# quinnchr-personal/Continuum-Mechanics-MFEM

Measured on AMD Instinct MI355X. Metric: DoF-iter/s (CG, 3D p=2 hex convection-diffusion) + achieved HBM GB/s, higher is better.
Workload: dtype f64; 1 GPU; 64x64x64 hex, H1 p=2, PA D+C+M (kinds=7), Jacobi-CG 100 it/step; dofs=2146689, elements=262144, parallelism=single, series=weak: an n^3 slab per rank

## Files before the change

### continuum-mechanics-mfem_amd/csrc/brick_core.hpp

```cpp
#pragma once
#include <hip/hip_runtime.h>

#include <cstdint>
#include <type_traits>

#include "pa_core.hpp"

#ifndef CDFEM_PS8_SKIP
#define CDFEM_PS8_SKIP 1
#endif

namespace cdfem {

struct BrickGeom {
    int nbx, nby, nbz;
    int Lx, Ly, Lz;
    int xcd;
    int bz0, bzs;
    const uint8_t *bess;
    int stag = 0, stag_round = 0;
};

__device__ __forceinline__ void brick_stagger(const BrickGeom &g)
{
// ... 45 lines not shown
template <int S, int STEP = 64>
struct LatWalk {
    int x, y, z;
    uint32_t gid;
    __device__ __forceinline__ LatWalk(unsigned t, uint32_t g0, uint32_t Lx, uint32_t Lxy)
        : x((int)(t % S)), y((int)((t / S) % S)), z((int)(t / (S * S)))
    {
        gid = g0 + (uint32_t)x + Lx * (uint32_t)y + Lxy * (uint32_t)z;
    }
    __device__ __forceinline__ void next(uint32_t dgid, uint32_t cxd, uint32_t cyd)
    {
        constexpr int dx = STEP % S, dy = (STEP / S) % S, dz = STEP / (S * S);
        x += dx;
        const int cx = x >= S ? 1 : 0;
        x -= S & -cx;
        y += dy + cx;
        const int cy = y >= S ? 1 : 0;
        y -= S & -cy;
        z += dz + cy;
        gid += dgid + (cxd & (uint32_t)-cx) + (cyd & (uint32_t)-cy);
    }
};

template <int B, int E, typename F>
__device__ __forceinline__ void static_for(F &&f)
{
    if constexpr (B < E) {
        f(std::integral_constant<int, B>{});
        static_for<B + 1, E>(f);
    }
}

__device__ __forceinline__ int opaque(int v)
{
    asm volatile("" : "+v"(v));
    return v;
}

template <int S, int SZ = S>
__device__ __forceinline__ double patch_sum8(__amdgpu_buffer_rsrc_t bp, const BrickGeom &g, int gx, int gy, int gz)
{
    constexpr int s1 = S - 1, sz1 = SZ - 1;
    const int qx = min(gx / s1, g.nbx - 1), qy = min(gy / s1, g.nby - 1), qz = min(gz / sz1, g.nbz - 1);
    const int px = gx - qx * s1, py = gy - qy * s1, pz = gz - qz * sz1;
    const bool fx = px == 0 && qx > 0, fy = py == 0 && qy > 0, fz = pz == 0 && qz > 0;
    const uint32_t R = (uint32_t)g.nbx * S, A = (uint32_t)g.nby * S * R;
// ... 42 lines not shown
```

### continuum-mechanics-mfem_amd/csrc/brick_kernels.hip

```cpp
#include <hip/hip_runtime.h>

#include <type_traits>
#include <vector>
#include <algorithm>
#include <cmath>

#include "cdfem_internal.hpp"
#include "brick_core.hpp"
#include "pa_core.hpp"
#include "reduce.hpp"

#ifndef CDFEM_BRICK_LDS
#define CDFEM_BRICK_LDS 1
#endif

namespace cdfem {

__device__ __forceinline__ int bsel(bool c, int a, int b)
{
    const int m = -(int)c;
    return (a & m) | (b & ~m);
}
template <int S>
__device__ __forceinline__ int face_index(int a, int b, int c)
// ... 580 lines not shown
    }
    den = wave_sum(den);
    if (grp <= 1) {
        if (t == 0) part[b] = den;
        return;
    }
    const int gi = b / grp, g0 = gi * grp, gn = min(grp, nbrick - g0);
    uint32_t prev = 0;
    if (t == 0) {
        __hip_atomic_store(&part[b], den, __ATOMIC_RELAXED, __HIP_MEMORY_SCOPE_AGENT);
        asm volatile("s_waitcnt vmcnt(0)" ::: "memory");
        prev = __hip_atomic_fetch_add(&gcnt[gi], 1u, __ATOMIC_RELAXED, __HIP_MEMORY_SCOPE_AGENT);
    }
    prev = (uint32_t)__shfl((int)prev, 0, 64);
    if (prev != (uint32_t)(gn - 1)) return;
    double v = t < gn ? __hip_atomic_load(&part[g0 + t], __ATOMIC_RELAXED, __HIP_MEMORY_SCOPE_AGENT) : 0.0;
    v = wave_sum(v);
    if (t == 0) {
        gsum[gi] = v;
        __hip_atomic_store(&gcnt[gi], 0u, __ATOMIC_RELAXED, __HIP_MEMORY_SCOPE_AGENT);
    }
}

template <int S, bool XF, bool PB = false, bool DS = false, bool EP = false, int SZ = S>
__global__ void __launch_bounds__(kRedThreads)
k_cg_update_faces(double *__restrict__ x, double *__restrict__ r, const double *__restrict__ d,
                  const double *__restrict__ dinv, const double *__restrict__ pb,
                  const uint8_t *__restrict__ ess, const BrickGeom g,
                  const FastDiv fdx, const FastDiv fdxy, int zlo_shared,
                  const double *__restrict__ remote_lo, const double *__restrict__ remote_hi,
                  double *__restrict__ part, KrylovState *__restrict__ st, int den_step,
                  const double *__restrict__ apart, int napart)
{
    constexpr int s1 = S - 1, sz1 = SZ - 1;
    constexpr uint32_t PV = (uint32_t)S * S * SZ;
    __shared__ double sh[kRedThreads / 64 + 1];
    if (st->done) return;
    double alpha = 0.0;
    if constexpr (DS) {
        const double den = sum_partials_all<16>(apart, napart, sh);
        if (blockIdx.x == 0 && threadIdx.x == 0) cg_den_step(st, den);
        if (den == 0.0) return;
        alpha = st->betanom / den;
    } else if (den_step) {
        const double den = st->red[0];
        if (blockIdx.x == 0 && threadIdx.x == 0) cg_den_step(st, den);
        if (den == 0.0) return;
        alpha = st->betanom / den;
    } else {
        alpha = st->alpha;
    }
    const int n = g.Lx * g.Ly * g.Lz;
    const int plane = g.Lx * g.Ly;
    double acc = 0.0;
    if constexpr (EP) {
        static_assert(PB, "EP reads the patch buffer with the predicated loads");
        const auto bp = brsrc(pb, 8u * (uint32_t)g.nbx * g.nby * g.nbz * PV);
        for (int gid = blockIdx.x * blockDim.x + threadIdx.x; gid < n; gid += gridDim.x * blockDim.x) {
            const int gz = (int)fdiv((uint32_t)gid, fdxy);
            const int rem = gid - gz * plane;
            const int gy = (int)fdiv((uint32_t)rem, fdx);
            const int gx = rem - gy * g.Lx;
            const double rold = r[gid], mi = dinv[gid];
            const double xi = XF ? 0.0 : x[gid], di = XF ? 0.0 : d[gid];
            double qi = patch_sum8<S, SZ>(bp, g, gx, gy, gz);
            if (remote_lo && gz == 0) qi += remote_lo[rem];
            if (remote_hi && gz == g.Lz - 1) qi += remote_hi[rem];
            if constexpr (!XF) __builtin_nontemporal_store(xi + alpha * di, &x[gid]);
            const double ri = rold - alpha * qi;
            __builtin_nontemporal_store(ri, &r[gid]);
            if (!(zlo_shared && gz == 0)) acc += ri * (mi * ri);
        }
    } else {
        for (int gid = blockIdx.x * blockDim.x + threadIdx.x; gid < n; gid += gridDim.x * blockDim.x) {
            const int gz = (int)fdiv((uint32_t)gid, fdxy);
            const int rem = gid - gz * plane;
            const int gy = (int)fdiv((uint32_t)rem, fdx);
            const int gx = rem - gy * g.Lx;
            const bool is_ess = ess[gid] != 0;
            const double di = (!XF || is_ess) ? d[gid] : 0.0, xi = XF ? 0.0 : x[gid];
            const double rold = r[gid], mi = dinv[gid];
            double qi;
            if constexpr (PB) {
                qi = patch_sum8<S, SZ>(brsrc(pb, 8u * (uint32_t)g.nbx * g.nby * g.nbz * PV), g, gx, gy, gz);
            } else if (gx % s1 == 0 || gy % s1 == 0 || gz % sz1 == 0) {
                int bxs[2], pxs[2], nxc = 0, bys[2], pys[2], nyc = 0, bzs[2], pzs[2], nzc = 0;
                const int qx = gx / s1, qy = gy / s1, qz = gz / sz1;
                if (gx - qx * s1 == 0) {
                    if (qx - 1 >= 0) { bxs[nxc] = qx - 1; pxs[nxc] = s1; ++nxc; }
                    if (qx < g.nbx) { bxs[nxc] = qx; pxs[nxc] = 0; ++nxc; }
                } else { bxs[0] = qx; pxs[0] = gx - qx * s1; nxc = 1; }
                if (gy - qy * s1 == 0) {
                    if (qy - 1 >= 0) { bys[nyc] = qy - 1; pys[nyc] = s1; ++nyc; }
                    if (qy < g.nby) { bys[nyc] = qy; pys[nyc] = 0; ++nyc; }
                } else { bys[0] = qy; pys[0] = gy - qy * s1; nyc = 1; }
                if (gz - qz * sz1 == 0) {
                    if (qz - 1 >= 0) { bzs[nzc] = qz - 1; pzs[nzc] = sz1; ++nzc; }
                    if (qz < g.nbz) { bzs[nzc] = qz; pzs[nzc] = 0; ++nzc; }
                } else { bzs[0] = qz; pzs[0] = gz - qz * sz1; nzc = 1; }
                qi = 0.0;
                for (int kz = 0; kz < nzc; ++kz)
                    for (int ky = 0; ky < nyc; ++ky)
                        for (int kx = 0; kx < nxc; ++kx) {
                            qi += pb[patch_idx<S, SZ>(g, bxs[kx], bys[ky], bzs[kz], pxs[kx], pys[ky], pzs[kz])];
// ... 431 lines not shown
    BrickRun edge{0, c->nbz - 1, 2, s}, inner{1, 1, c->nbz - 2, c->stream};
    if (bfkk >= 0) {
        edge.kk = inner.kk = bfkk;
        edge.nupart = inner.nupart = cg_den_fold_grid(c);
    }
    const hipError_t e = brick_cg2_run(c, r, dinv, d_old, d_new, q, edge, x);
    if (e != hipSuccess) return e;
    return brick_cg2_run(c, r, dinv, d_old, d_new, q, inner, x);
}

hipError_t launch_cg_update_faces(cdfem_ctx *c, double *x, double *r, const double *q, const double *d,
                                  const double *dinv, const double *remote_lo, const double *remote_hi,
                                  bool den_step, bool xfold)
{
    const BrickGeom g = geom_of(c);
    const FastDiv fdx = make_fastdiv((uint32_t)c->Lx), fdxy = make_fastdiv((uint32_t)(c->Lx * c->Ly));
    const int64_t need = (c->nl + kRedThreads - 1) / kRedThreads;
    const unsigned grid = (unsigned)(need < 16384 ? need : 16384);
    const bool ds = !den_step && cg_den_fold_on(c);
    const unsigned ugrid = ds ? (unsigned)cg_den_fold_grid(c) : grid;
    double *const upart = ds ? c->d_part + c->nblk : c->d_part;
    const double *const apart = c->den_grp > 1 ? c->d_gsum : c->d_part;
    const int napart = c->den_grp > 1 ? den_parts(c) : c->nblk;
#define CDFEM_UPD4(S_, XF_, PB_, DS_, EP_)                                                                 \
    hipLaunchKernelGGL((k_cg_update_faces<S_, XF_, PB_, DS_, EP_, SZ_>), dim3(ugrid), dim3(kRedThreads), 0, c->stream, x, \
                       r, d, dinv, c->d_face, c->d_ess, g, fdx, fdxy, c->zlo_shared, remote_lo, remote_hi, upart, \
                       c->d_state, (int)den_step, apart, napart)
    const bool ep = pa_af(c) == 2 && c->p <= 2;
#define CDFEM_UPD3(S_, XF_, PB_, DS_)                                                                      \
    if (ep && PB_) { CDFEM_UPD4(S_, XF_, PB_, DS_, PB_); } else { CDFEM_UPD4(S_, XF_, PB_, DS_, false); }
#define CDFEM_UPD2(S_, XF_, PB_)                                                                           \
    if (ds) { CDFEM_UPD3(S_, XF_, PB_, true); } else { CDFEM_UPD3(S_, XF_, PB_, false); }
    const bool pb = c->brick_upd_pb != 0 && brick_fits(c);
#define CDFEM_UPD(S_)                                                                                       \
    if (xfold) {                                                                                            \
        if (pb) { CDFEM_UPD2(S_, true, true); } else { CDFEM_UPD2(S_, true, false); }                       \
    } else {                                                                                                \
        if (pb) { CDFEM_UPD2(S_, false, true); } else { CDFEM_UPD2(S_, false, false); }                     \
    }
    if (c->p == 1) {
        constexpr int SZ_ = kBrick * 1 + 1;
        CDFEM_UPD(kBrick * 1 + 1);
    } else if (c->p == 2 || (c->p == 4 && c->hb_ez == 2)) {
        constexpr int SZ_ = kBrick * 2 + 1;
        CDFEM_UPD(kBrick * 2 + 1);
    } else if (c->p == 4 && c->hb_ez == 4) {
        constexpr int SZ_ = 4 * 4 + 1;
        CDFEM_UPD(kHoBrickEdge * 4 + 1);
    } else if (c->p == 3 && c->hb_ez == 2) {
        constexpr int SZ_ = kHoBrickEdge * 3 + 1;
        CDFEM_UPD(kHoBrickEdge * 3 + 1);
    } else if (c->p == 3 && c->hb_ez == 4) {
        constexpr int SZ_ = 4 * 3 + 1;
        CDFEM_UPD(kHoBrickEdge * 3 + 1);
    } else {
        return hipErrorInvalidValue;
// ... 81 lines not shown
```

### continuum-mechanics-mfem_amd/csrc/brick_um.hip

```cpp
#include <hip/hip_runtime.h>

#include <algorithm>
#include <cmath>
#include <vector>

#include "cdfem_internal.hpp"
#include "brick_core.hpp"
#include "pa_core.hpp"
#include "reduce.hpp"

#ifndef CDFEM_BUM_ADD
#define CDFEM_BUM_ADD 0
#endif

namespace cdfem {

constexpr int kUmSlots = 32, kUmN = 27;
constexpr int kUmRow[kUmSlots] = {0,  1,  4,  3,  2,  7,  22, 5,  6,  19, 10, 21, 8,  25, 16, 23,
                                  18, 9,  12, 13, 20, 11, 14, -1, 24, 15, -1, -1, 26, 17, -1, -1};
constexpr int um_class(int l) { return (l % 3 & 1) | ((l / 3 % 3 & 1) << 1) | ((l / 9 & 1) << 2); }
constexpr bool um_row_order_ok()
{
    int seen[kUmN] = {};
    for (int g = 0; g < kUmSlots / 4; ++g) {
// ... 5 lines not shown
            if (l >= kUmN || seen[l]++) return false;
            if (cls & (1 << um_class(l))) return false;
            cls |= 1 << um_class(l);
        }
    }
    for (int l = 0; l < kUmN; ++l)
        if (!seen[l]) return false;
    return true;
}
static_assert(um_row_order_ok(), "kUmRow: every dof once, one class once per group of 4 slots");

template <int G>
__device__ __forceinline__ int um_slot_off(int kg)
{
    constexpr int S = 9;
    auto off = [](int l) constexpr { return l < 0 ? -1 : (l / 9) * S * S + (l / 3 % 3) * S + l % 3; };
    constexpr int o0 = off(kUmRow[4 * G]), o1 = off(kUmRow[4 * G + 1]), o2 = off(kUmRow[4 * G + 2]),
                  o3 = off(kUmRow[4 * G + 3]);
    return kg == 0 ? o0 : kg == 1 ? o1 : kg == 2 ? o2 : o3;
}
template <int G>
constexpr bool um_group_padded() { return kUmRow[4 * G + 1] < 0 || kUmRow[4 * G + 2] < 0 || kUmRow[4 * G + 3] < 0; }

template <bool XF, bool BF, bool FULL>
__global__ void __launch_bounds__(64, 2)
k_brick_cg(const double *__restrict__ r, const double *__restrict__ dinv, const double *__restrict__ d_old,
           double *__restrict__ d_new, double *__restrict__ face, const double *__restrict__ amat,
           const uint8_t *__restrict__ ess, const BrickGeom g, int zlo_shared, double *__restrict__ part,
           KrylovState *__restrict__ st, double *__restrict__ x, const double *__restrict__ upart, int nupart,
           int kk, double *__restrict__ gsum, uint32_t *__restrict__ gcnt, int grp, int nbrick)
{
    constexpr int P = 2, S = kBrick * P + 1, S2 = S * S, S3 = S * S * S, NDE = kUmN;
    static_assert(S == 9, "um_slot_off is written for the 9^3 patch");
    __shared__ double s_in[S3];
    __shared__ double s_out[S3];
    if (st->done) return;
    brick_stagger(g);
    double beta = st->beta;
    constexpr int NPL = 16;
    double pv[NPL];
    if constexpr (BF) {
        if (kk > 0) {
            const auto bu = brsrc(upart, 8u * (uint32_t)nupart);
#pragma unroll
            for (int i = 0; i < NPL; ++i) pv[i] = bload(bu, 8u * ((uint32_t)threadIdx.x + 64u * i));
        }
    }
    const double alpha_prev = XF ? st->alpha : 0.0;
    const int t = threadIdx.x;
    const int bl = brick_id(g), nxy = g.nbx * g.nby;
    const int bz = g.bz0 + (bl / nxy) * g.bzs;
    const int b = bl % nxy + nxy * bz;
    const int bx = b % g.nbx, by = (b / g.nbx) % g.nby;
    const int gx0 = (S - 1) * bx, gy0 = (S - 1) * by, gz0 = (S - 1) * bz;
    const bool lastx = bx == g.nbx - 1, lasty = by == g.nby - 1, lastz = bz == g.nbz - 1;
    double den = 0.0;
    constexpr int NI = (S3 + 63) / 64;
    const int Lx = g.Lx, Lxy = g.Lx * g.Ly;
    const uint32_t nl = (uint32_t)Lxy * (uint32_t)g.Lz;
    const auto br = brsrc(r, 8u * nl), bm = brsrc(dinv, 8u * nl), bo = brsrc(d_old, 8u * nl);
    const auto be = brsrc(ess, nl), bd = brsrc(d_new, 8u * nl), bxf = brsrc(x, XF ? 8u * nl : 0u);
    double rv[NI], mv[NI], ov[NI], xv[NI];
    uint32_t woffv[NI];
    uint32_t dbits = 0, ebits = 0;
    uint8_t ev[NI];
    double dev[NI];
    const uint32_t uLx = (uint32_t)Lx, uLxy = (uint32_t)Lxy;
    constexpr uint32_t wdx = 64 % S, wdy = (64 / S) % S, wdz = 64 / (S * S);
    const uint32_t dgid = wdx + wdy * uLx + wdz * uLxy, cxd = uLx - S, cyd = uLxy - S * uLx;
    LatWalk<S> pw0(t, (uint32_t)gx0 + uLx * (uint32_t)gy0 + uLxy * (uint32_t)gz0, uLx, uLxy);
    auto gather = [&](auto kc) {
        constexpr int k = decltype(kc)::value;
        const unsigned i = t + 64 * k;
        const int px = pw0.x, py = pw0.y, pz = pw0.z;
        const uint32_t gid = pw0.gid;
        pw0.next(dgid, cxd, cyd);
        const int gz = gz0 + pz;
        const bool in = i < S3 && (FULL || (gx0 + px < g.Lx && gy0 + py < g.Ly && gz < g.Lz));
        const uint32_t off = in ? 8u * gid : kOOB;
        rv[k] = bload(br, off);
        mv[k] = bload(bm, off);
        ov[k] = bload(bo, off);
        ev[k] = __builtin_amdgcn_raw_buffer_load_b8(be, in ? gid : kOOB, 0, 0);
        const bool writer = in && (px < S - 1 || lastx) && (py < S - 1 || lasty) && (pz < S - 1 || lastz);
        woffv[k] = writer ? off : kOOB;
        dbits |= (uint32_t)(writer && !(zlo_shared && gz == 0)) << k;
        if constexpr (XF) xv[k] = bload(bxf, woffv[k]);
    };
    auto form = [&](auto kc) {
        constexpr int k = decltype(kc)::value;
        const unsigned i = t + 64 * k;
        if (k == NI - 1 && i >= S3) return;
        const double dn = mv[k] * rv[k] + beta * ov[k];
        const bool e = ev[k] != 0;
        bstore(bd, woffv[k], dn);
        if constexpr (XF) bstore(bxf, woffv[k], xv[k] + alpha_prev * ov[k]);
        den += (e && ((dbits >> k) & 1u)) ? dn * dn : 0.0;
        s_in[i] = e ? 0.0 : dn;
        s_out[i] = 0.0;
        ebits |= (uint32_t)e << k;
        dev[k] = ((dbits >> k) & 1u) ? dn : 0.0;
    };
    static_for<0, NI>(gather);
    if constexpr (BF) {
        if (kk > 0) {
            double v = 0.0;
#pragma unroll
            for (int q = 0; q < NPL; ++q) v += pv[q];
            const double B = wave_sum(v);
            const bool stop = cg_stop_kind(st, B, kk) != kCgGoOn;
            if (b == 0 && t == 0) {
#ifdef CDFEM_DEBUG
                assert(st->iter == kk);
#endif
                cg_update_logic_at(st, B, kk);
            }
            if (stop) return;
            beta = B / st->nom;
        }
    }
    static_for<0, NI>(form);
    __syncthreads();

    {
        const int n16 = t & 15, kg = t >> 4;
        double av[2][7];
#pragma unroll
        for (int mt = 0; mt < 2; ++mt)
#pragma unroll
            for (int ks = 0; ks < 7; ++ks) av[mt][ks] = amat[(mt * 7 + ks) * 64 + t];
        const int ob0 = P * (n16 >> 2) * S + P * (n16 & 3);
        const bool vxy = FULL || (gx0 + P * (n16 & 3) + P < g.Lx && gy0 + P * (n16 >> 2) + P < g.Ly);
        auto node_off = [&](int j) { return (j / 9) * S2 + ((j / 3) % 3) * S + j % 3; };
        v4d_t acc[2][4];
#pragma unroll
        for (int mt = 0; mt < 2; ++mt)
#pragma unroll
            for (int nt = 0; nt < 4; ++nt) acc[mt][nt] = v4d_t{0.0, 0.0, 0.0, 0.0};
#pragma unroll
        for (int ks = 0; ks < 7; ++ks) {
            const int j = 4 * ks + kg;
            const int jo = node_off(j < NDE ? j : 0);
#pragma unroll
// ... 64 lines not shown
        __hip_atomic_store(&part[b], den, __ATOMIC_RELAXED, __HIP_MEMORY_SCOPE_AGENT);
        asm volatile("s_waitcnt vmcnt(0)" ::: "memory");
        prev = __hip_atomic_fetch_add(&gcnt[gi], 1u, __ATOMIC_RELAXED, __HIP_MEMORY_SCOPE_AGENT);
    }
    prev = (uint32_t)__shfl((int)prev, 0, 64);
    if (prev != (uint32_t)(gn - 1)) return;
    double v = t < gn ? __hip_atomic_load(&part[g0 + t], __ATOMIC_RELAXED, __HIP_MEMORY_SCOPE_AGENT) : 0.0;
    v = wave_sum(v);
    if (t == 0) {
        gsum[gi] = v;
        __hip_atomic_store(&gcnt[gi], 0u, __ATOMIC_RELAXED, __HIP_MEMORY_SCOPE_AGENT);
    }
}

hipError_t launch_brick_um(cdfem_ctx *c, const BrickGeom &g, unsigned nbrick_launch, hipStream_t s, bool whole,
                           const double *r, const double *dinv, const double *d_old, double *d_new, double *x, int kk,
                           int nupart)
{
    if (c->d_uelem == nullptr || c->p != 2) return hipErrorInvalidValue;
    const dim3 grid(nbrick_launch), block(64);
    const double *upart = c->d_part + c->nblk;
    double *const dpart = c->den_out ? c->den_out : c->d_part;
    const bool full = c->sx % kBrick == 0 && c->sy % kBrick == 0 && c->sz % kBrick == 0;
#define CDFEM_BUM(XF_, BF_, FU_)                                                                              \
    do {                                                                                                      \
        if (whole)                                                                                            \
            CDFEM_LAUNCH(c, (k_brick_cg<XF_, BF_, FU_>), grid, block, 0, r, dinv, d_old, d_new, c->d_face,      \
                         c->d_uelem, c->d_ess, g, c->zlo_shared, dpart, c->d_state, x, upart, nupart, kk,       \
                         c->d_gsum, c->d_gcnt, c->den_grp, c->nblk);                                            \
        else                                                                                                  \
            hipLaunchKernelGGL((k_brick_cg<XF_, BF_, FU_>), grid, block, 0, s, r, dinv, d_old, d_new, c->d_face, \
                               c->d_uelem, c->d_ess, g, c->zlo_shared, dpart, c->d_state, x, upart, nupart, kk, \
                               c->d_gsum, c->d_gcnt, c->den_grp, c->nblk);                                      \
    } while (0)
#define CDFEM_BUM2(XF_, BF_)                                                                                  \
    do {                                                                                                      \
        if (full) CDFEM_BUM(XF_, BF_, true);                                                                  \
        else CDFEM_BUM(XF_, BF_, false);                                                                      \
    } while (0)
    if (kk >= 0) {
        if (x) CDFEM_BUM2(true, true);
        else CDFEM_BUM2(false, true);
    } else {
        if (x) CDFEM_BUM2(true, false);
        else CDFEM_BUM2(false, false);
    }
#undef CDFEM_BUM2
#undef CDFEM_BUM
    return hipGetLastError();
}

__global__ void __launch_bounds__(256)
k_uniform_check(const double *__restrict__ gaff, const int32_t *__restrict__ perm, int nslots, int nc, int ne,
                double tol, int *__restrict__ bad)
{
    const int s = blockIdx.x * blockDim.x + threadIdx.x;
    if (s >= nslots) return;
    const int e = perm[s];
    if (e < 0 || e >= ne) return;
    const size_t b = (size_t)(s / kLanes), lane = (size_t)(s % kLanes);
    bool diff = false;
    for (int k = 0; k < nc; ++k) diff |= fabs(gaff[(b * nc + k) * kLanes + lane] - gaff[(size_t)k * kLanes]) > tol;
    if (diff) *bad = 1;
}

template <int D1, int Q1, unsigned K>
__global__ void __launch_bounds__(64)
k_uniform_elem(const double *__restrict__ gaff, const Tab<D1, Q1> T, double *__restrict__ A)
{
    constexpr int N = D1 * D1 * D1;
// ... 49 lines not shown
        if (e == hipSuccess) e = hipStreamSynchronize(c->stream);
    }
    const hipError_t ef = hipFree(scratch);
    if (e != hipSuccess) return e;
    if (ef != hipSuccess) return ef;
    if (hbad) return hipSuccess;
    for (int mt = 0; mt < 2; ++mt)
        for (int ks = 0; ks < 7; ++ks)
            for (int l = 0; l < 64; ++l) {
                const int i = kUmRow[16 * mt + (l & 15)], j = 4 * ks + (l >> 4);
                op[(mt * 7 + ks) * 64 + l] = (i >= 0 && j < N) ? h[i * N + j] : 0.0;
            }
    void *d = nullptr;
    if ((e = hipMalloc(&d, sizeof(double) * op.size())) != hipSuccess) return e;
    e = hipMemcpy(d, op.data(), sizeof(double) * op.size(), hipMemcpyHostToDevice);
    if (e != hipSuccess) {
        (void)hipFree(d);
        return e;
    }
    c->d_uelem = static_cast<double *>(d);
    return hipSuccess;
}

}
```

### continuum-mechanics-mfem_amd/csrc/capi.hip

```cpp
#include <hip/hip_runtime.h>

#include <algorithm>
#include <chrono>
#include <cmath>
#include <cstdio>
#include <cstdlib>
#include <cstring>
#include <limits>
#include <new>
#include <stdexcept>
#include <string>
#include <vector>

#include "cdfem_internal.hpp"
#include "brick_core.hpp"

using namespace cdfem;

namespace {

struct HipError : std::runtime_error {
    explicit HipError(const std::string &m) : std::runtime_error(m) {}
};
struct ArgError : std::runtime_error {
// ... 83 lines not shown
                for (int k = 0; k < dim; ++k)
                    if (v >> k & 1) p += X[(1 << k) * dim + i] - X[i];
                if (std::fabs(p - X[v * dim + i]) > tol) return false;
            }
        }
    }
    return true;
}

void free_mesh(cdfem_ctx *c)
{
    dfree(c->d_verts); dfree(c->d_map); dfree(c->d_e2l_off); dfree(c->d_e2l_pos);
    dfree(c->d_ess); dfree(c->d_ess_list); dfree(c->d_qd); dfree(c->d_qaff); dfree(c->d_geom); dfree(c->d_hgeom); dfree(c->d_Ye); dfree(c->d_dinv);
    for (auto &w : c->d_w) dfree(w);
    dfree(c->d_part); dfree(c->d_tpart); dfree(c->d_gm); dfree(c->d_gm_part); dfree(c->d_ktab);
    c->ktab_key = -1;
    dfree(c->d_perm); dfree(c->d_face); dfree(c->d_ones); dfree(c->d_dalt);
    for (auto &b : c->d_if) dfree(b);
    dfree(c->d_stab); dfree(c->d_stab_lf); dfree(c->d_rowptr); dfree(c->d_cols); dfree(c->d_diagpos); dfree(c->d_coff);
    dfree(c->d_cpos); dfree(c->d_vals); dfree(c->d_vals_c); dfree(c->d_Ee);
    dfree(c->d_sptr); dfree(c->d_srows); dfree(c->d_scols); dfree(c->d_smap); dfree(c->d_sdel); dfree(c->d_svals);
    dfree(c->d_swide);
    dfree(c->d_uelem);
    dfree(c->d_hoelem);
    c->d_sdel = nullptr;
    c->d_swide = nullptr;
    c->sell_nnz_wide = 0;
    dfree(c->d_hptr); dfree(c->d_hidx); dfree(c->d_sloc);
    c->d_hptr = c->d_hidx = nullptr;
    c->d_sloc = nullptr;
    c->lds_rows = 0;
    c->lds_max = 0;
    c->sell_lpr = 1;
    dfree(c->d_rperm); dfree(c->d_pv[0]); dfree(c->d_pv[1]); dfree(c->d_dinv_p);
    c->d_rperm = nullptr; c->d_pv[0] = c->d_pv[1] = nullptr; c->d_dinv_p = nullptr;
    dfree(c->d_svals_c);
    c->d_svals_c = nullptr;
    dfree(c->d_lfq);
    c->lfq_cap = 0;
    ilu_free(c);
    partition_free(c);
    c->nslices = c->nstored = 0;
    c->sell_windowed = false;
    c->geom = 0;
    c->fa_ready = false;
    c->nnz = 0;
// ... 209 lines not shown
void dev_out(cdfem_ctx *c, double *dst, int where, const double *dsrc, size_t n)
{
    if (where == CDFEM_DEVICE) {
        if (dst != dsrc)
            HIPCHK(hipMemcpyAsync(dst, dsrc, n * sizeof(double), hipMemcpyDeviceToDevice, c->stream));
        return;
    }
    HIPCHK(hipMemcpyAsync(dst, dsrc, n * sizeof(double), hipMemcpyDeviceToHost, c->stream));
    HIPCHK(hipStreamSynchronize(c->stream));
}

void ensure_dinv(cdfem_ctx *c)
{
    if (c->dinv_ready) return;
    double *diag = c->d_w[7];
    if (c->fa_ready) {
        HIPCHK(launch_csr_diag(c, diag));
    } else {
        HIPCHK(launch_diag_elem(c, c->d_Ye));
        HIPCHK(launch_e2l(c, c->d_Ye, nullptr, diag, false, 0));
    }
    interface_sum(c, diag);
    HIPCHK(launch_dinv(c, diag, c->d_dinv));
    c->dinv_ready = true;
}

const double *solver_dinv(cdfem_ctx *c)
{
    ensure_dinv(c);
    if (!c->perm_space) return c->d_dinv;
    if (!c->d_dinv_p) c->d_dinv_p = dalloc<double>(c->nl);
    HIPCHK(launch_perm(c, true, c->d_dinv, c->d_dinv_p));
    return c->d_dinv_p;
}

bool mr_fold_agreed(cdfem_ctx *c)
{
    const double ok = cg_mr_fold(c) ? 1.0 : 0.0, nb = den_parts(c), ng = cg_den_fold_grid(c);
    double h[5] = {ok, nb, nb * nb, ng, ng * ng};
    if (!c->d_small) c->d_small = dalloc<double>(8);
    HIPCHK(hipMemcpyAsync(c->d_small, h, sizeof(h), hipMemcpyHostToDevice, c->stream));
    comm_allreduce(c, c->d_small, 5);
    HIPCHK(hipMemcpyAsync(h, c->d_small, sizeof(h), hipMemcpyDeviceToHost, c->stream));
    HIPCHK(hipStreamSynchronize(c->stream));
    const double n = c->nranks;
    return h[0] == n && h[2] * n == h[1] * h[1] && h[4] * n == h[3] * h[3];
// ... 1364 lines not shown
        const std::string k(key);
        if (k == "brick_xcd") {
            if (value < 0 || value > 1) throw ArgError("brick_xcd must be 0 or 1");
            c->brick_xcd = value;
        } else if (k == "brick_byte_limit") {
            if (value < 0) throw ArgError("brick_byte_limit must be 0 (the default 2^31) or 1..2^31-1");
            c->brick_limit = value == 0 ? (int64_t)1 << 31 : value;
        } else if (k == "den_group") {
            if (value < 0 || value > 64 || (value & (value - 1)) != 0)
                throw ArgError("den_group must be 0 (automatic) or a power of two up to 64");
            c->den_group_opt = value;
        } else if (k == "cg_mr_fold") {
            if (value != 0 && value != 1) throw ArgError("cg_mr_fold must be 0 or 1");
            c->cg_mr_fold = value;
        } else if (k == "ho_brick_mfma") {
            if (value != 0 && value != 1) throw ArgError("ho_brick_mfma must be 0 or 1");
            c->ho_brick_mfma = value;
        } else if (k == "brick_stagger") {
            if (value < -1 || value > 511) throw ArgError("brick_stagger must be -1 (automatic), 0 (off) or 1..511");
            c->brick_stagger = value;
        } else if (k == "pa_uniform") {
            if (value != 0 && value != 1) throw ArgError("pa_uniform must be 0 or 1");
            c->pa_uniform = value;
        } else if (k == "ho_uniform") {
            if (value != 0 && value != 1) throw ArgError("ho_uniform must be 0 or 1");
            c->ho_uniform = value;
        } else if (k == "ho_uniform_grid") {
            if (value < 0) throw ArgError("ho_uniform_grid must be 0 (automatic) or the number of workgroups");
            c->ho_uniform_grid = value;
        } else if (k == "brick_mfma") {
            if (value != 0 && value != 1) throw ArgError("brick_mfma must be 0 or 1");
            c->brick_mfma = value;
        } else if (k == "ho_block_z") {
            if (value != 2 && value != 4) throw ArgError("ho_block_z must be 2 or 4");
            c->ho_block_z = value;
        } else if (k == "ho_brick") {
            if (value != 0 && value != 1) throw ArgError("ho_brick must be 0 or 1");
            c->ho_brick = value;
        } else if (k == "mr_overlap") {
            if (value < 0 || value > 1) throw ArgError("mr_overlap must be 0 or 1");
            c->mr_overlap = value;
        } else if (k == "brick_mult_pb") {
            if (value != 0 && value != 1) throw ArgError("brick_mult_pb must be 0 or 1");
            c->brick_mult_pb = value;
        } else if (k == "cg_beta_fold") {
            if (value != 0 && value != 1) throw ArgError("cg_beta_fold must be 0 or 1");
// ... 214 lines not shown
            const bool xf = c->cg_xfold != 0;
            const double nrow = 16.0 * ((c->nd + 15) / 16), ncol = 4.0 * ((c->nd + 3) / 4);
            const double fac = ho_uniform_elem(c) ? 8.0 * nrow * ncol : 8.0 * c->ncomp * ne;
            *bytes = k == CDFEM_K_APPLY ? fac + 33.0 * nl + patches + (xf ? 16.0 * nl : 0.0)
                                        : (xf ? 25.0 : 49.0) * nl + patches;
            return CDFEM_OK;
        }
        if (use_brick(c)) {
            const int64_t s1 = (int64_t)kBrick * c->p;
            int64_t nface_dofs = 0;
            for (int64_t z = 0; z < c->Lz; ++z)
                for (int64_t y = 0; y < c->Ly; ++y) {
                    if (z % s1 == 0 || y % s1 == 0) { nface_dofs += c->Lx; continue; }
                    nface_dofs += (c->Lx - 1) / s1 + 1;
                }
            const double nf = (double)nface_dofs;
            const double S = kBrick * c->p + 1.0;
            const double patches = 8.0 * S * S * S * (double)c->nblk;
            const bool xf = c->cg_xfold != 0 && pa_af(c) == 2;
            switch (k) {
            case CDFEM_K_APPLY:
                *bytes = (uniform_elem(c) ? 8.0 * 14 * 64
                          : pa_geom_on(c) ? 8.0 * GeomLayout::kNC * ne
                                          : 8.0 * c->ncomp * (c->d_qaff ? 1.0 : nq) * ne) + 24.0 * nl +
                         1.0 * nl + 8.0 * nl + patches + (xf ? 16.0 * nl : 0.0);
                return CDFEM_OK;
            case CDFEM_K_E2L:
                *bytes = (c->brick_mult_pb && pa_af(c) == 2) ? patches + 9.0 * nl
                                                             : 8.0 * c->nface * (double)c->nblk + 25.0 * nf;
                return CDFEM_OK;
            case CDFEM_K_UPDATE:
                *bytes = (xf ? 25.0 : 49.0) * nl + patches;
                return CDFEM_OK;
            default: throw ArgError("kernel not launched on the brick path");
            }
        }
        const double nqs = (c->qlay == 1 ? tile_affine(c) : (c->dim == 3 && c->d_qaff != nullptr)) ? 1.0 : nq;
        const bool hgeo = c->qlay == 1 && ho_geom_on(c);
        switch (k) {
        case CDFEM_K_APPLY:
            if (c->epencil)
                *bytes = 9.0 * nl + (hgeo ? 8.0 * HoGeomLayout::kNC * ne : 8.0 * c->ncomp * nqs * ne) + 8.0 * nd * ne +
                         (tile_dfold_ok(c) ? 16.0 * nl : 0.0);
            else
                *bytes = 8.0 * nl + (c->qlay == 0 && c->dim == 3 && pa_geom_on(c) ? 8.0 * GeomLayout::kNC * ne
                                     : hgeo                                       ? 8.0 * HoGeomLayout::kNC * ne
                                                                                  : 8.0 * c->ncomp * nqs * ne) +
                         4.0 * nd * ne + 8.0 * nd * ne;
            break;
        case CDFEM_K_E2L:
            if (c->epencil)
                *bytes = 8.0 * nd * ne + 1.0 * nl + 8.0 * nl + 8.0 * nl;
            else
                *bytes = 8.0 * nd * ne + 4.0 * nd * ne + 4.0 * nl + 8.0 * nl + 8.0 * nl;
            break;
// ... 10 lines not shown
```

### continuum-mechanics-mfem_amd/csrc/cdfem_internal.hpp

```cpp
#pragma once
#include <hip/hip_ext.h>
#include <hip/hip_runtime.h>

#include <cstdint>
#include <string>
#include <vector>

#include "../../include/cdfem.h"

namespace cdfem {

constexpr int kLanes = 64;
constexpr int kMaxD1 = 6;
constexpr int kMaxQ1 = 8;

struct Rule1D {
    int d1 = 0, q1 = 0;
    double B[kMaxQ1][kMaxD1] = {};
    double G[kMaxQ1][kMaxD1] = {};
    double pts[kMaxQ1] = {};
    double wts[kMaxQ1] = {};
};

void gll_nodes(int p, double *x);
// ... 87 lines not shown
    std::vector<uint8_t> h_ess;

    bool structured = false;
    bool epencil = false;
    int sx = 0, sy = 0, sz = 0;
    int nbx = 0, nby = 0, nbz = 0;
    int hb_nbx = 0, hb_nby = 0, hb_nbz = 0, hb_nblk = 0;
    int ho_block_z = 2;
    int hb_ez = 2;
    uint8_t *d_bess = nullptr;
    int ho_brick = 1;
    double *d_hbpart = nullptr;
    double *den_out = nullptr;
    int den_grp = 1;
    int den_group_opt = 0;
    double *d_gsum = nullptr;
    uint32_t *d_gcnt = nullptr;
    int64_t gsum_cap = 0;
    int ho_brick_mfma = 0;
    int brick_stagger = -1;
    int brick_mfma = 0;
    int pa_uniform = 1;
    double *d_uelem = nullptr;
    int ho_uniform = 0;
    int ho_uniform_grid = 0;
    double *d_hoelem = nullptr;
    int hoelem_p = 0;
    unsigned hoelem_kinds = 0;
    int64_t Lx = 0, Ly = 0, Lz = 0;
    double *d_face = nullptr;
    double *d_ones = nullptr;
    double *d_dalt = nullptr;
    int nface = 0;
    int gm_ept = 0;
    int gm_ept_auto = 4;
    int gm_pb = 1;
    int gm_poll = 4;
    int64_t gm_ept_n = -1;
    int brick_xcd = 1;
    int64_t brick_limit = (int64_t)1 << 31;
    int64_t slab_nl_max = 0, slab_nb_max = 0;
    int ncu = 0;
    int zlo_shared = 0;
    int zhi_shared = 0;
    cdfem::Comm *comm = nullptr;
    int rank = 0, nranks = 1;
// ... 113 lines not shown
            (c)->ext_ev[0] = (c)->ext_ev[1] = nullptr;                                                       \
        } else {                                                                                             \
            hipLaunchKernelGGL(kernel, grid, block, shm, (c)->stream, __VA_ARGS__);                          \
        }                                                                                                    \
    } while (0)

namespace cdfem {

inline bool tile_affine(const cdfem_ctx *c)
{
    if (c->d_qaff == nullptr) return false;
    if (c->ho_mfma == 0) return true;
    return c->kinds == 7 && (c->ho_mfma == 1 || c->ho_mfma == 8 || c->ho_mfma == 9);
}
inline bool tile_kron(const cdfem_ctx *c) { return c->d_qaff != nullptr && c->ho_mfma == 0 && c->pa_affine == 2; }
inline int pa_af(const cdfem_ctx *c) { return c->d_qaff == nullptr ? 0 : (c->pa_affine == 2 ? 2 : 1); }
inline bool pa_geom_on(const cdfem_ctx *c) { return c->d_geom != nullptr && c->pa_geom != 0 && c->d_qaff == nullptr; }
inline bool ho_geom_on(const cdfem_ctx *c)
{
    return c->d_hgeom != nullptr && c->ho_geom != 0 && c->d_qaff == nullptr && c->ho_mfma == 0;
}
inline int pa_form(const cdfem_ctx *c) { return pa_geom_on(c) ? 3 : pa_af(c); }
inline bool uniform_elem(const cdfem_ctx *c) { return c->d_uelem != nullptr && c->pa_uniform != 0 && pa_af(c) == 2; }

hipError_t launch_setup_qdata(cdfem_ctx *c, const double *d_kappa_q, const double *d_kmat_q, double kappa, double alpha,
                              const double *conv, const double *d_conv_q, const double *d_mass_q,
                              double mass);
hipError_t launch_setup_geom(cdfem_ctx *c);
hipError_t launch_setup_hgeom(cdfem_ctx *c);
hipError_t launch_apply(cdfem_ctx *c, const double *x, double *Ye, bool constrained);
hipError_t launch_apply_wpe(cdfem_ctx *c, const double *x, double *Ye, bool con, const KrylovState *st);
hipError_t launch_apply_st(cdfem_ctx *c, const double *x, double *Ye, bool constrained,
                           const KrylovState *st);
hipError_t launch_diag_elem(cdfem_ctx *c, double *Ye);
hipError_t launch_lf_elem(cdfem_ctx *c, const double *d_fq, double *Ye);
hipError_t launch_quad_points(cdfem_ctx *c, const Rule1D &r, double *xyz);
bool apply_supported(int dim, int p);

constexpr int kBrick = 4;
constexpr int kHoBrickEdge = 2;
bool brick_supported(int dim, int p);
int brick_count(const cdfem_ctx *c);
int brick_patch_side(const cdfem_ctx *c);
int brick_patch_side_z(const cdfem_ctx *c);
bool cg_den_fold_on(const cdfem_ctx *c);
bool cg_mr_fold(const cdfem_ctx *c);
// ... 5 lines not shown
hipError_t ho_ktab(cdfem_ctx *c, const double **out);
bool brick_fits(const cdfem_ctx *c);
hipError_t launch_brick_mult(cdfem_ctx *c, const double *x, double *y, bool constrained, int which);


hipError_t launch_e2l(cdfem_ctx *c, const double *Ye, const double *x, double *y, bool constrained,
                      int cg_mode);
hipError_t launch_set_ess(cdfem_ctx *c, double *y, const double *x);
hipError_t launch_mask_ess(cdfem_ctx *c, const double *x, double *y);
hipError_t launch_axpby(cdfem_ctx *c, double a, const double *x, double b, double *y);
hipError_t launch_axpby_n(cdfem_ctx *c, int64_t n, double a, const double *x, double b, double *y);
hipError_t launch_dinv(cdfem_ctx *c, const double *diag, double *dinv);
hipError_t launch_cg_init(cdfem_ctx *c, const double *B, double *x, double *r, double *z, double *d,
                          const double *dinv, double rel_tol, double abs_tol, int max_iter);
hipError_t launch_cg_update(cdfem_ctx *c, double *x, double *r, double *z, const double *d,
                            const double *dinv);
hipError_t launch_cg_direction(cdfem_ctx *c, const double *z, double *d);
hipError_t launch_cg_update_noz(cdfem_ctx *c, double *x, double *r, const double *q, const double *d,
                                const double *dinv);
hipError_t launch_zero(cdfem_ctx *c, double *y);
hipError_t launch_den_fin(cdfem_ctx *c, int nparts);
hipError_t launch_update_fin(cdfem_ctx *c, int nparts, int64_t off = 0);
hipError_t setup_uniform_elem(cdfem_ctx *c);
hipError_t setup_ho_uniform_elem(cdfem_ctx *c);
bool ho_uniform_path(const cdfem_ctx *c);
bool ho_uniform_elem(const cdfem_ctx *c);
hipError_t launch_brick_cg2(cdfem_ctx *c, const double *r, const double *dinv, const double *d_old,
                            double *d_new, double *q, double *x = nullptr, int bfkk = -1);
int cg_den_fold_grid(const cdfem_ctx *c);
bool cg_beta_fold_ok(const cdfem_ctx *c);
hipError_t launch_cg_xflush(cdfem_ctx *c, double *x, const double *d0, const double *d1);
hipError_t launch_cg_update_faces(cdfem_ctx *c, double *x, double *r, const double *q, const double *d,
                                  const double *dinv, const double *remote_lo, const double *remote_hi,
                                  bool den_step = false, bool xfold = false);
hipError_t launch_dot(cdfem_ctx *c, const double *a, const double *b, double *d_out);
hipError_t launch_den_local(cdfem_ctx *c, const double *d, const double *q);

void comm_destroy(cdfem_ctx *c);
void comm_allreduce(cdfem_ctx *c, double *dbuf, int n);
void comm_exchange(cdfem_ctx *c, const double *send_lo, double *recv_lo, const double *send_hi,
                   double *recv_hi, int64_t n, hipStream_t s = nullptr);
void interface_sum(cdfem_ctx *c, double *v);
void interface_copy_owner(cdfem_ctx *c, double *v);
void comm_exchange_nbr_buf(cdfem_ctx *c, const std::vector<int64_t> &off, const double *dsend, double *drecv,
                           hipStream_t s = nullptr);
void partition_free(cdfem_ctx *c);
// ... 88 lines not shown
```

Measured before the change: 43.36 billion DoF-iter/s.

## Replace per-DoF Jacobi inverse diagonal reads with a 64-entry class table

On a uniform structured p=2 mesh the inverse diagonal depends only on each DoF's position class per axis (low boundary, high boundary, even, odd). A setup pass builds and checks a 64-entry table. The brick CG and face-update kernels then look up dinv from shared memory by computing the class from coordinates, instead of streaming an 8-byte-per-DoF array. This cuts HBM traffic in a bandwidth-bound CG iteration, at the cost of extra index arithmetic, a shared-memory table with a barrier, and a validation kernel with a tolerance check at setup.

```diff
diff --git a/continuum-mechanics-mfem_amd/csrc/brick_core.hpp b/continuum-mechanics-mfem_amd/csrc/brick_core.hpp
--- a/continuum-mechanics-mfem_amd/csrc/brick_core.hpp
+++ b/continuum-mechanics-mfem_amd/csrc/brick_core.hpp
@@ -91,6 +91,8 @@
     }
 };
 
+__host__ __device__ __forceinline__ int udiag_class(int g, int L) { return g == 0 ? 2 : g == L - 1 ? 3 : g & 1; }
+
 template <int B, int E, typename F>
 __device__ __forceinline__ void static_for(F &&f)
 {
diff --git a/continuum-mechanics-mfem_amd/csrc/brick_kernels.hip b/continuum-mechanics-mfem_amd/csrc/brick_kernels.hip
--- a/continuum-mechanics-mfem_amd/csrc/brick_kernels.hip
+++ b/continuum-mechanics-mfem_amd/csrc/brick_kernels.hip
@@ -626,7 +626,7 @@
     }
 }
 
-template <int S, bool XF, bool PB = false, bool DS = false, bool EP = false, int SZ = S>
+template <int S, bool XF, bool PB = false, bool DS = false, bool EP = false, int SZ = S, bool UD = false>
 __global__ void __launch_bounds__(kRedThreads)
 k_cg_update_faces(double *__restrict__ x, double *__restrict__ r, const double *__restrict__ d,
                   const double *__restrict__ dinv, const double *__restrict__ pb,
@@ -639,7 +639,11 @@
     constexpr int s1 = S - 1, sz1 = SZ - 1;
     constexpr uint32_t PV = (uint32_t)S * S * SZ;
     __shared__ double sh[kRedThreads / 64 + 1];
+    __shared__ double s_tab[UD ? kUdiagN : 1];
+    static_assert(!UD || kRedThreads >= kUdiagN, "UD: one table entry per thread");
     if (st->done) return;
+    double tabv = 0.0;
+    if constexpr (UD) tabv = threadIdx.x < kUdiagN ? dinv[threadIdx.x] : 0.0;
     double alpha = 0.0;
     if constexpr (DS) {
         const double den = sum_partials_all<16>(apart, napart, sh);
@@ -657,6 +661,10 @@
     const int n = g.Lx * g.Ly * g.Lz;
     const int plane = g.Lx * g.Ly;
     double acc = 0.0;
+    if constexpr (UD) {
+        if (threadIdx.x < kUdiagN) s_tab[threadIdx.x] = tabv;
+        __syncthreads();
+    }
     if constexpr (EP) {
         static_assert(PB, "EP reads the patch buffer with the predicated loads");
         const auto bp = brsrc(pb, 8u * (uint32_t)g.nbx * g.nby * g.nbz * PV);
@@ -665,7 +673,15 @@
             const int rem = gid - gz * plane;
             const int gy = (int)fdiv((uint32_t)rem, fdx);
             const int gx = rem - gy * g.Lx;
-            const double rold = r[gid], mi = dinv[gid];
+            const double rold = r[gid];
+            double mi;
+            if constexpr (UD) {
+                const bool is_ess = ess[gid] != 0;
+                const double tv = s_tab[udiag_class(gx, g.Lx) + 4 * udiag_class(gy, g.Ly) + 16 * udiag_class(gz, g.Lz)];
+                mi = is_ess ? 1.0 : tv;
+            } else {
+                mi = dinv[gid];
+            }
             const double xi = XF ? 0.0 : x[gid], di = XF ? 0.0 : d[gid];
             double qi = patch_sum8<S, SZ>(bp, g, gx, gy, gz);
             if (remote_lo && gz == 0) qi += remote_lo[rem];
@@ -683,7 +699,14 @@
             const int gx = rem - gy * g.Lx;
             const bool is_ess = ess[gid] != 0;
             const double di = (!XF || is_ess) ? d[gid] : 0.0, xi = XF ? 0.0 : x[gid];
-            const double rold = r[gid], mi = dinv[gid];
+            const double rold = r[gid];
+            double mi;
+            if constexpr (UD) {
+                const double tv = s_tab[udiag_class(gx, g.Lx) + 4 * udiag_class(gy, g.Ly) + 16 * udiag_class(gz, g.Lz)];
+                mi = is_ess ? 1.0 : tv;
+            } else {
+                mi = dinv[gid];
+            }
             double qi;
             if constexpr (PB) {
                 qi = patch_sum8<S, SZ>(brsrc(pb, 8u * (uint32_t)g.nbx * g.nby * g.nbz * PV), g, gx, gy, gz);
@@ -1161,16 +1184,22 @@
     double *const upart = ds ? c->d_part + c->nblk : c->d_part;
     const double *const apart = c->den_grp > 1 ? c->d_gsum : c->d_part;
     const int napart = c->den_grp > 1 ? den_parts(c) : c->nblk;
-#define CDFEM_UPD4(S_, XF_, PB_, DS_, EP_)                                                                 \
-    hipLaunchKernelGGL((k_cg_update_faces<S_, XF_, PB_, DS_, EP_, SZ_>), dim3(ugrid), dim3(kRedThreads), 0, c->stream, x, \
+#define CDFEM_UPD4(S_, XF_, PB_, DS_, EP_, UD_)                                                               \
+    hipLaunchKernelGGL((k_cg_update_faces<S_, XF_, PB_, DS_, EP_, SZ_, UD_>), dim3(ugrid), dim3(kRedThreads), 0, c->stream, x, \
                        r, d, dinv, c->d_face, c->d_ess, g, fdx, fdxy, c->zlo_shared, remote_lo, remote_hi, upart, \
                        c->d_state, (int)den_step, apart, napart)
+    const bool pb = c->brick_upd_pb != 0 && brick_fits(c);
     const bool ep = pa_af(c) == 2 && c->p <= 2;
+    const bool ud = uniform_diag(c) && dinv == c->d_dinv && c->p == 2;
+    if (ud) dinv = c->d_udiag;
 #define CDFEM_UPD3(S_, XF_, PB_, DS_)                                                                      \
-    if (ep && PB_) { CDFEM_UPD4(S_, XF_, PB_, DS_, PB_); } else { CDFEM_UPD4(S_, XF_, PB_, DS_, false); }
+    if (ep && PB_) {                                                                                       \
+        if (ud) { CDFEM_UPD4(S_, XF_, PB_, DS_, PB_, (S_ == 9 && SZ_ == 9)); }                             \
+        else { CDFEM_UPD4(S_, XF_, PB_, DS_, PB_, false); }                                                \
+    } else if (ud) { CDFEM_UPD4(S_, XF_, PB_, DS_, false, (S_ == 9 && SZ_ == 9)); }                        \
+    else { CDFEM_UPD4(S_, XF_, PB_, DS_, false, false); }
 #define CDFEM_UPD2(S_, XF_, PB_)                                                                           \
     if (ds) { CDFEM_UPD3(S_, XF_, PB_, true); } else { CDFEM_UPD3(S_, XF_, PB_, false); }
-    const bool pb = c->brick_upd_pb != 0 && brick_fits(c);
 #define CDFEM_UPD(S_)                                                                                       \
     if (xfold) {                                                                                            \
         if (pb) { CDFEM_UPD2(S_, true, true); } else { CDFEM_UPD2(S_, true, false); }                       \
diff --git a/continuum-mechanics-mfem_amd/csrc/brick_um.hip b/continuum-mechanics-mfem_amd/csrc/brick_um.hip
--- a/continuum-mechanics-mfem_amd/csrc/brick_um.hip
+++ b/continuum-mechanics-mfem_amd/csrc/brick_um.hip
@@ -51,7 +51,7 @@
 template <int G>
 constexpr bool um_group_padded() { return kUmRow[4 * G + 1] < 0 || kUmRow[4 * G + 2] < 0 || kUmRow[4 * G + 3] < 0; }
 
-template <bool XF, bool BF, bool FULL>
+template <bool XF, bool BF, bool FULL, bool UD>
 __global__ void __launch_bounds__(64, 2)
 k_brick_cg(const double *__restrict__ r, const double *__restrict__ dinv, const double *__restrict__ d_old,
            double *__restrict__ d_new, double *__restrict__ face, const double *__restrict__ amat,
@@ -63,6 +63,7 @@
     static_assert(S == 9, "um_slot_off is written for the 9^3 patch");
     __shared__ double s_in[S3];
     __shared__ double s_out[S3];
+    __shared__ double s_tab[UD ? kUdiagN + 1 : 1];
     if (st->done) return;
     brick_stagger(g);
     double beta = st->beta;
@@ -87,9 +88,20 @@
     constexpr int NI = (S3 + 63) / 64;
     const int Lx = g.Lx, Lxy = g.Lx * g.Ly;
     const uint32_t nl = (uint32_t)Lxy * (uint32_t)g.Lz;
-    const auto br = brsrc(r, 8u * nl), bm = brsrc(dinv, 8u * nl), bo = brsrc(d_old, 8u * nl);
+    const auto br = brsrc(r, 8u * nl), bm = brsrc(dinv, UD ? 8u * kUdiagN : 8u * nl), bo = brsrc(d_old, 8u * nl);
     const auto be = brsrc(ess, nl), bd = brsrc(d_new, 8u * nl), bxf = brsrc(x, XF ? 8u * nl : 0u);
-    double rv[NI], mv[NI], ov[NI], xv[NI];
+    double rv[NI], mv[UD ? 1 : NI], ov[NI], xv[NI];
+    uint32_t cw[UD ? (NI + 2) / 3 : 1] = {};
+    uint32_t wx = 0, wy = 0, wz = 0;
+    if constexpr (UD) {
+        auto axis_word = [](int b0, int e) {
+            return 0x4444u | (b0 == 0 ? 2u : 0u) | (e < S ? 3u << (2 * e) : 0u);
+        };
+        wx = axis_word(bx, g.Lx - 1 - gx0);
+        wy = axis_word(by, g.Ly - 1 - gy0);
+        wz = axis_word(bz, g.Lz - 1 - gz0);
+        mv[0] = bload(bm, 8u * (uint32_t)t);
+    }
     uint32_t woffv[NI];
     uint32_t dbits = 0, ebits = 0;
     uint8_t ev[NI];
@@ -108,7 +120,13 @@
         const bool in = i < S3 && (FULL || (gx0 + px < g.Lx && gy0 + py < g.Ly && gz < g.Lz));
         const uint32_t off = in ? 8u * gid : kOOB;
         rv[k] = bload(br, off);
-        mv[k] = bload(bm, off);
+        if constexpr (UD) {
+            const uint32_t cl = ((wx >> (2 * px)) & 3u) | (((wy >> (2 * py)) & 3u) << 2) | (((wz >> (2 * pz)) & 3u) << 4);
+            cw[k / 3] |= cl << (9 * (k % 3) + 3);
+            asm volatile("" : "+v"(cw[k / 3]));
+        } else {
+            mv[k] = bload(bm, off);
+        }
         ov[k] = bload(bo, off);
         ev[k] = __builtin_amdgcn_raw_buffer_load_b8(be, in ? gid : kOOB, 0, 0);
         const bool writer = in && (px < S - 1 || lastx) && (py < S - 1 || lasty) && (pz < S - 1 || lastz);
@@ -120,8 +138,15 @@
         constexpr int k = decltype(kc)::value;
         const unsigned i = t + 64 * k;
         if (k == NI - 1 && i >= S3) return;
-        const double dn = mv[k] * rv[k] + beta * ov[k];
         const bool e = ev[k] != 0;
+        double m;
+        if constexpr (UD) {
+            const uint32_t o = e ? 8u * kUdiagN : (cw[k / 3] >> (9 * (k % 3))) & (8u * (kUdiagN - 1));
+            m = *reinterpret_cast<const double *>(reinterpret_cast<const char *>(s_tab) + o);
+        } else {
+            m = mv[k];
+        }
+        const double dn = m * rv[k] + beta * ov[k];
         bstore(bd, woffv[k], dn);
         if constexpr (XF) bstore(bxf, woffv[k], xv[k] + alpha_prev * ov[k]);
         den += (e && ((dbits >> k) & 1u)) ? dn * dn : 0.0;
@@ -148,6 +173,11 @@
             beta = B / st->nom;
         }
     }
+    if constexpr (UD) {
+        s_tab[t] = mv[0];
+        if (t == 0) s_tab[kUdiagN] = 1.0;
+        __syncthreads();
+    }
     static_for<0, NI>(form);
     __syncthreads();
 
@@ -258,21 +288,28 @@
     const double *upart = c->d_part + c->nblk;
     double *const dpart = c->den_out ? c->den_out : c->d_part;
     const bool full = c->sx % kBrick == 0 && c->sy % kBrick == 0 && c->sz % kBrick == 0;
-#define CDFEM_BUM(XF_, BF_, FU_)                                                                              \
+    const bool ud = uniform_diag(c) && dinv == c->d_dinv;
+    if (ud) dinv = c->d_udiag;
+#define CDFEM_BUM(XF_, BF_, FU_, UD_)                                                                              \
     do {                                                                                                      \
         if (whole)                                                                                            \
-            CDFEM_LAUNCH(c, (k_brick_cg<XF_, BF_, FU_>), grid, block, 0, r, dinv, d_old, d_new, c->d_face,      \
+            CDFEM_LAUNCH(c, (k_brick_cg<XF_, BF_, FU_, UD_>), grid, block, 0, r, dinv, d_old, d_new, c->d_face,      \
                          c->d_uelem, c->d_ess, g, c->zlo_shared, dpart, c->d_state, x, upart, nupart, kk,       \
                          c->d_gsum, c->d_gcnt, c->den_grp, c->nblk);                                            \
         else                                                                                                  \
-            hipLaunchKernelGGL((k_brick_cg<XF_, BF_, FU_>), grid, block, 0, s, r, dinv, d_old, d_new, c->d_face, \
+            hipLaunchKernelGGL((k_brick_cg<XF_, BF_, FU_, UD_>), grid, block, 0, s, r, dinv, d_old, d_new, c->d_face, \
                                c->d_uelem, c->d_ess, g, c->zlo_shared, dpart, c->d_state, x, upart, nupart, kk, \
                                c->d_gsum, c->d_gcnt, c->den_grp, c->nblk);                                      \
     } while (0)
+#define CDFEM_BUM3(XF_, BF_, FU_)                                                                             \
+    do {                                                                                                      \
+        if (ud) CDFEM_BUM(XF_, BF_, FU_, true);                                                               \
+        else CDFEM_BUM(XF_, BF_, FU_, false);                                                                 \
+    } while (0)
 #define CDFEM_BUM2(XF_, BF_)                                                                                  \
     do {                                                                                                      \
-        if (full) CDFEM_BUM(XF_, BF_, true);                                                                  \
-        else CDFEM_BUM(XF_, BF_, false);                                                                      \
+        if (full) CDFEM_BUM3(XF_, BF_, true);                                                                 \
+        else CDFEM_BUM3(XF_, BF_, false);                                                                     \
     } while (0)
     if (kk >= 0) {
         if (x) CDFEM_BUM2(true, true);
@@ -282,6 +319,7 @@
         else CDFEM_BUM2(false, false);
     }
 #undef CDFEM_BUM2
+#undef CDFEM_BUM3
 #undef CDFEM_BUM
     return hipGetLastError();
 }
@@ -377,4 +415,89 @@
     return hipSuccess;
 }
 
-}
+__device__ __forceinline__ int udiag_index(int gid, int Lx, int Ly, int Lz)
+{
+    const int gx = gid % Lx, gy = (gid / Lx) % Ly, gz = gid / (Lx * Ly);
+    return udiag_class(gx, Lx) + 4 * udiag_class(gy, Ly) + 16 * udiag_class(gz, Lz);
+}
+
+__global__ void __launch_bounds__(256)
+k_udiag_first(const uint8_t *__restrict__ ess, int Lx, int Ly, int Lz, uint32_t *__restrict__ first)
+{
+    __shared__ uint32_t lo[kUdiagN];
+    if (threadIdx.x < kUdiagN) lo[threadIdx.x] = ~0u;
+    __syncthreads();
+    const int n = Lx * Ly * Lz;
+    for (int gid = blockIdx.x * blockDim.x + threadIdx.x; gid < n; gid += gridDim.x * blockDim.x)
+        if (!ess[gid]) atomicMin(&lo[udiag_index(gid, Lx, Ly, Lz)], (uint32_t)gid);
+    __syncthreads();
+    if (threadIdx.x < kUdiagN && lo[threadIdx.x] != ~0u) atomicMin(&first[threadIdx.x], lo[threadIdx.x]);
+}
+
+__global__ void __launch_bounds__(kUdiagN)
+k_udiag_fill(const double *__restrict__ dinv, const uint32_t *__restrict__ first, double *__restrict__ tab)
+{
+    const uint32_t f = first[threadIdx.x];
+    tab[threadIdx.x] = f != ~0u ? dinv[f] : 1.0;
+}
+
+__global__ void __launch_bounds__(256)
+k_udiag_check(const double *__restrict__ dinv, const uint8_t *__restrict__ ess, const double *__restrict__ tab,
+              int Lx, int Ly, int Lz, double tol, int *__restrict__ flags)
+{
+    const int n = Lx * Ly * Lz;
+    bool bad = false, inexact = false;
+    for (int gid = blockIdx.x * blockDim.x + threadIdx.x; gid < n; gid += gridDim.x * blockDim.x) {
+        const double m = dinv[gid];
+        if (ess[gid]) {
+            bad |= m != 1.0;
+        } else {
+            const double tv = tab[udiag_index(gid, Lx, Ly, Lz)];
+            bad |= !(fabs(m - tv) <= tol * fabs(tv));
+            inexact |= m != tv;
+        }
+    }
+    if (bad) flags[0] = 1;
+    if (inexact) flags[1] = 1;
+}
+
+hipError_t setup_uniform_diag(cdfem_ctx *c)
+{
+    hipError_t e = hipSuccess;
+    if (c->d_udiag) {
+        e = hipFree(c->d_udiag);
+        c->d_udiag = nullptr;
+        if (e != hipSuccess) return e;
+    }
+    c->udiag_bitwise = false;
+    if (c->d_uelem == nullptr || !c->structured || c->dim != 3 || c->p != 2 || c->perm_space ||
+        c->nl != c->Lx * c->Ly * c->Lz || c->nl >= ((int64_t)1 << 31))
+        return hipSuccess;
+    void *buf = nullptr;
+    if ((e = hipMalloc(&buf, sizeof(double) * kUdiagN + sizeof(uint32_t) * (kUdiagN + 2))) != hipSuccess) return e;
+    double *tab = static_cast<double *>(buf);
+    uint32_t *first = reinterpret_cast<uint32_t *>(tab + kUdiagN);
+    int *flags = reinterpret_cast<int *>(first + kUdiagN);
+    int hflags[2] = {1, 1};
+    const int Lx = (int)c->Lx, Ly = (int)c->Ly, Lz = (int)c->Lz;
+    const dim3 grid((unsigned)std::min<int64_t>((c->nl + 255) / 256, 1024)), block(256);
+    e = hipMemsetAsync(first, 0xff, sizeof(uint32_t) * kUdiagN, c->stream);
+    if (e == hipSuccess) e = hipMemsetAsync(flags, 0, 2 * sizeof(int), c->stream);
+    if (e == hipSuccess) {
+        hipLaunchKernelGGL(k_udiag_first, grid, block, 0, c->stream, c->d_ess, Lx, Ly, Lz, first);
+        hipLaunchKernelGGL(k_udiag_fill, dim3(1), dim3(kUdiagN), 0, c->stream, c->d_dinv, first, tab);
+        hipLaunchKernelGGL(k_udiag_check, grid, block, 0, c->stream, c->d_dinv, c->d_ess, tab, Lx, Ly, Lz, 1e-14, flags);
+        e = hipGetLastError();
+    }
+    if (e == hipSuccess) e = hipMemcpyAsync(hflags, flags, sizeof(hflags), hipMemcpyDeviceToHost, c->stream);
+    if (e == hipSuccess) e = hipStreamSynchronize(c->stream);
+    if (e != hipSuccess || hflags[0]) {
+        const hipError_t ef = hipFree(buf);
+        return e != hipSuccess ? e : ef;
+    }
+    c->d_udiag = tab;
+    c->udiag_bitwise = hflags[1] == 0;
+    return hipSuccess;
+}
+
+}
diff --git a/continuum-mechanics-mfem_amd/csrc/capi.hip b/continuum-mechanics-mfem_amd/csrc/capi.hip
--- a/continuum-mechanics-mfem_amd/csrc/capi.hip
+++ b/continuum-mechanics-mfem_amd/csrc/capi.hip
@@ -129,6 +129,7 @@
     dfree(c->d_sptr); dfree(c->d_srows); dfree(c->d_scols); dfree(c->d_smap); dfree(c->d_sdel); dfree(c->d_svals);
     dfree(c->d_swide);
     dfree(c->d_uelem);
+    dfree(c->d_udiag);
     dfree(c->d_hoelem);
     c->d_sdel = nullptr;
     c->d_swide = nullptr;
@@ -384,6 +385,17 @@
     }
     interface_sum(c, diag);
     HIPCHK(launch_dinv(c, diag, c->d_dinv));
+    HIPCHK(setup_uniform_diag(c));
+    if (multi_rank(c)) {
+        const double mine = c->d_udiag ? 1.0 : 0.0;
+        double all = mine;
+        if (!c->d_small) c->d_small = dalloc<double>(8);
+        HIPCHK(hipMemcpyAsync(c->d_small, &mine, sizeof(double), hipMemcpyHostToDevice, c->stream));
+        comm_allreduce(c, c->d_small, 1);
+        HIPCHK(hipMemcpyAsync(&all, c->d_small, sizeof(double), hipMemcpyDeviceToHost, c->stream));
+        HIPCHK(hipStreamSynchronize(c->stream));
+        if (all != (double)c->nranks) dfree(c->d_udiag);
+    }
     c->dinv_ready = true;
 }
 
@@ -1794,6 +1806,9 @@
         } else if (k == "pa_uniform") {
             if (value != 0 && value != 1) throw ArgError("pa_uniform must be 0 or 1");
             c->pa_uniform = value;
+        } else if (k == "pa_uniform_diag") {
+            if (value != 0 && value != 1) throw ArgError("pa_uniform_diag must be 0 or 1");
+            c->pa_uniform_diag = value;
         } else if (k == "ho_uniform") {
             if (value != 0 && value != 1) throw ArgError("ho_uniform must be 0 or 1");
             c->ho_uniform = value;
@@ -2054,15 +2069,16 @@
             case CDFEM_K_APPLY:
                 *bytes = (uniform_elem(c) ? 8.0 * 14 * 64
                           : pa_geom_on(c) ? 8.0 * GeomLayout::kNC * ne
-                                          : 8.0 * c->ncomp * (c->d_qaff ? 1.0 : nq) * ne) + 24.0 * nl +
-                         1.0 * nl + 8.0 * nl + patches + (xf ? 16.0 * nl : 0.0);
+                                          : 8.0 * c->ncomp * (c->d_qaff ? 1.0 : nq) * ne) +
+                         (uniform_diag(c) ? 16.0 * nl + 8.0 * kUdiagN : 24.0 * nl) + 1.0 * nl + 8.0 * nl + patches +
+                         (xf ? 16.0 * nl : 0.0);
                 return CDFEM_OK;
             case CDFEM_K_E2L:
                 *bytes = (c->brick_mult_pb && pa_af(c) == 2) ? patches + 9.0 * nl
                                                              : 8.0 * c->nface * (double)c->nblk + 25.0 * nf;
                 return CDFEM_OK;
             case CDFEM_K_UPDATE:
-                *bytes = (xf ? 25.0 : 49.0) * nl + patches;
+                *bytes = (xf ? 25.0 : 49.0) * nl + patches - (uniform_diag(c) ? 8.0 * nl : 0.0);
                 return CDFEM_OK;
             default: throw ArgError("kernel not launched on the brick path");
             }
diff --git a/continuum-mechanics-mfem_amd/csrc/cdfem_internal.hpp b/continuum-mechanics-mfem_amd/csrc/cdfem_internal.hpp
--- a/continuum-mechanics-mfem_amd/csrc/cdfem_internal.hpp
+++ b/continuum-mechanics-mfem_amd/csrc/cdfem_internal.hpp
@@ -133,6 +133,9 @@
     int brick_mfma = 0;
     int pa_uniform = 1;
     double *d_uelem = nullptr;
+    int pa_uniform_diag = 1;
+    double *d_udiag = nullptr;
+    bool udiag_bitwise = false;
     int ho_uniform = 0;
     int ho_uniform_grid = 0;
     double *d_hoelem = nullptr;
@@ -292,6 +295,11 @@
 }
 inline int pa_form(const cdfem_ctx *c) { return pa_geom_on(c) ? 3 : pa_af(c); }
 inline bool uniform_elem(const cdfem_ctx *c) { return c->d_uelem != nullptr && c->pa_uniform != 0 && pa_af(c) == 2; }
+constexpr int kUdiagN = 64;
+inline bool uniform_diag(const cdfem_ctx *c)
+{
+    return c->d_udiag != nullptr && c->dinv_ready && c->pa_uniform_diag != 0 && uniform_elem(c);
+}
 
 hipError_t launch_setup_qdata(cdfem_ctx *c, const double *d_kappa_q, const double *d_kmat_q, double kappa, double alpha,
                               const double *conv, const double *d_conv_q, const double *d_mass_q,
@@ -343,6 +351,7 @@
 hipError_t launch_den_fin(cdfem_ctx *c, int nparts);
 hipError_t launch_update_fin(cdfem_ctx *c, int nparts, int64_t off = 0);
 hipError_t setup_uniform_elem(cdfem_ctx *c);
+hipError_t setup_uniform_diag(cdfem_ctx *c);
 hipError_t setup_ho_uniform_elem(cdfem_ctx *c);
 bool ho_uniform_path(const cdfem_ctx *c);
 bool ho_uniform_elem(const cdfem_ctx *c);
```

Measured after the change: 45.33 billion DoF-iter/s, median of 6. +4.5%, better.
